# JuliaMLTools/GraphNets.jl

Measured on AMD Instinct MI355X. Metric: edges updated/sec, GNBlock fwd, 1M-edge batch, higher is better.
Workload: dtype f32; 1 GPU; C2: one shared Erdos-Renyi graph, 100k nodes / 1M edges, batch_size=1 (BASELINE configs[1]); dims=(10, 5, 0)=>(3, 4, 5), edges_whole_job=1000000, edges_per_gpu=1000000, nodes_per_gpu=100000, graphs_per_gpu=1, parallelism=single GPU

## Files before the change

graphnets.jl_amd/csrc/gnx_forward.hip:

```cpp
#include <algorithm>
#include <cstdlib>

#include "gnx_staging.h"
#include "gnx_step_hazard.h"

namespace gnx {

static_assert(GNX_ACT_IDENTITY == 0 && GNX_ACT_RELU == 1 && GNX_ACT_TANH == 2 && GNX_ACT_SIGMOID == 3 && GNX_ACT_GELU == 4,
              "act_apply (gnx_device.h) hard-codes the activation codes");

static int32_t check_block(const gnx_graphs* h, const gnx_block_params* p, int64_t R) {
  if (!h || !p) return fail(GNX_ERR_INVALID_ARG, "NULL handle or params");
  if (R <= 0) return fail(GNX_ERR_INVALID_ARG, "n_replicas must be >= 1");
  if (R > 1 && h->G != 1)
    return fail(GNX_ERR_INVALID_ARG, "n_replicas > 1 needs a single-graph handle (shared adjacency, batch.jl:66)");
  if (R > 65535) return fail(GNX_ERR_TOO_LARGE, "n_replicas exceeds the grid limit (65535)");
  const int d[6] = {p->de, p->dn, p->dg, p->oe, p->on, p->og};
  for (int i = 0; i < 6; ++i)
    if (d[i] < 0) return fail(GNX_ERR_DIMS, "negative feature width");
  if (p->de + p->dn + p->dg == 0) return fail(GNX_ERR_DIMS, "all input widths are 0 (gnblock.jl:48, batch.jl:56)");
  if (p->oe + p->on + p->og == 0) return fail(GNX_ERR_DIMS, "all output widths are 0 (gnblock.jl:49)");
  const gnx_dense* fn[3] = {&p->edgefn, &p->nodefn, &p->graphfn};
  const int out[3] = {p->oe, p->on, p->og};
  const int in[3] = {p->de + 2 * p->dn + p->dg, p->oe + p->dn + p->dg, p->oe + p->on + p->dg};
// ... 309 lines not shown
  int32_t rc = bf16 ? check_call(c) : GNX_OK;
  if (rc) return rc;
  if (prev && prev->workspace && (prev->workspace == c.ws || (c.p && c.p->og > 0 && prev->gf_out == c.gf_out)))
    return fail(GNX_ERR_INVALID_ARG, bf16 ? "internal: the pending step's workspace / gf_out is this step's"
                                          : "the pending call's workspace / gf_out must not be this call's (its graph update has not run yet)");
  bool took = false;
  rc = block_chained(c.on(c.s, GNX_PHASE_EDGE_NODE), prev, took);
  if (rc) return rc;
  if (took) {
    *pending = gnx_pending_update{c.ws, c.ws_bytes, static_cast<const float*>(c.gf), static_cast<float*>(c.gf_out)};
    return GNX_OK;
  }
  if (prev && prev->workspace) {
    rc = graph_update(c.h, c.p, c.elem, *prev, c.R, c.flags, c.s);
    if (rc) return rc;
  }
  *pending = gnx_pending_update{};
  return bf16 ? gnx_block_forward_typed(c.h, c.p, GNX_ELEM_BF16, c.ef, c.nf, c.gf, c.R, c.ef_out, c.nf_out, c.gf_out, c.ws, c.ws_bytes, c.flags, c.s) : block_plain(c);
}

int32_t gnx_block_forward_chained(const gnx_graphs* h, const gnx_block_params* p, const float* ef, const float* nf, const float* gf, int64_t R, float* ef_out,
                                  float* nf_out, float* gf_out, void* ws, size_t ws_bytes, uint32_t flags, void* stream, const gnx_pending_update* prev,
                                  gnx_pending_update* pending) {
  if (!pending) return fail(GNX_ERR_INVALID_ARG, "pending is NULL");
  DeviceTurn turn((hipStream_t)stream, p && matrix_core_widths(*p));
  if (flags & GNX_FLAG_DEFER_GRAPH_UPDATE) return fail(GNX_ERR_INVALID_ARG, "gnx_block_forward_chained defers the graph update itself");
  return chained_step(BlockCall{h, p, GNX_ELEM_F32, ef, nf, gf, R, ef_out, nf_out, gf_out, ws, ws_bytes, flags, (hipStream_t)stream, GNX_PHASE_ALL}, prev, pending);
}

static StepSpans step_spans(const gnx_graphs* h, const gnx_block_params* p, int64_t R, const gnx_block_step& st, size_t elem, size_t ws_extent) {
  const void* const in[3] = {st.ef, st.nf, st.gf};
  const void* const out[3] = {st.ef_out, st.nf_out, st.gf_out};
  const long long rows[3] = {(long long)h->E, (long long)h->N, (long long)h->G};
  const int in_w[3] = {p->de, p->dn, p->dg}, out_w[3] = {p->oe, p->on, p->og};
  return step_spans_of(in, out, st.workspace, st.workspace_bytes, rows, in_w, out_w, R, elem, ws_extent);
}

static bool steps_overlap_applies(const gnx_graphs* h, const gnx_block_params* p, int64_t R, uint32_t flags, hipStream_t s) {
  if (!h || !p || matrix_core_widths(*p) || (flags & GNX_FLAG_FORCE_GENERIC) || form(GNX_FLAG_NO_FORK) || profile_enabled()) return false;
  if (check_block(h, p, R) != GNX_OK) return false;
  return block_narrow_takes(h, block_probe(h, p), s);
}

constexpr int kStepsRunDefault = 8;
static_assert(kRunMax == kRunSlots, "gnx_step_hazard.h groups what gnx_device.h's table holds");
static int steps_run_max() {
  static const int v = [] {
    const char* e = getenv("GNX_STEPS_RUN_MAX");
    const int n = e && *e ? atoi(e) : kStepsRunDefault;
    return n < 1 ? 1 : (n > kRunMax ? kRunMax : n);
  }();
  return v;
}

static int32_t steps_schedule(const gnx_graphs* h, const gnx_block_params* p, int32_t elem, const gnx_block_step* steps, int64_t n_steps, int64_t R,
                              uint32_t flags, void* stream, bool overlap) {
  const AuxHold hold = overlap ? take_aux(h, true) : AuxHold{};
  const gnx_graphs::AuxSet* aux = hold.set;
  const bool two = aux != nullptr;
  hipStream_t str[2] = {(hipStream_t)stream, aux ? aux->stream : nullptr};
  gnx_pending_update pend[2]{};
  auto flush = [&](int k) -> int32_t {
    if (!pend[k].workspace) return GNX_OK;
    const int32_t rc = graph_update(h, p, elem, pend[k], R, flags, str[k]);
    pend[k] = gnx_pending_update{};
    return rc;
  };
  auto run = [&](const gnx_block_step& st, int k, gnx_pending_update* next) -> int32_t {
    const gnx_pending_update* prev = pend[k].workspace ? &pend[k] : nullptr;
    return chained_step(BlockCall{h, p, elem, st.ef, st.nf, st.gf, R, st.ef_out, st.nf_out, st.gf_out, st.workspace, st.workspace_bytes, flags, str[k], GNX_PHASE_ALL},
                        prev, next);
  };
  const bool bf16 = elem == GNX_ELEM_BF16;
  const bool valid = h && p && check_block(h, p, R) == GNX_OK;
  const size_t elem_bytes = bf16 ? 2 : sizeof(float);
  const size_t ws_extent = !valid ? 0 : bf16 ? typed_ws(h, p, R, true).total : block_ws(h, p, R).total;
  bool can_fuse = valid && R == 1 && !(flags & GNX_FLAG_FORCE_GENERIC) && steps_run_max() > 1 && !profile_enabled();
  auto slot_of = [&](const gnx_block_step& st, RunSlot& sl, BlockArgs* run_args) -> bool {
    Prepared q(BlockCall{h, p, elem, st.ef, st.nf, st.gf, R, st.ef_out, st.nf_out, st.gf_out, st.workspace, st.workspace_bytes, flags, str[0], GNX_PHASE_ALL});
    if (q.rc) return false;
    if (run_args) {
      if (!block_narrow_run_applies(h, q.a, bf16)) return can_fuse = false;
      *run_args = q.a;
    }
    sl = RunSlot{q.a.ef, q.a.nf, q.a.gf, q.a.ef_out, q.a.nf_out, q.a.gf_out, q.a.partials};
    return true;
  };
  if (two) {
    GNX_HIP(hipEventRecord(aux->fork, str[0]));
    GNX_HIP(hipStreamWaitEvent(str[1], aux->fork, 0));
  }
  RunSpans recent[3];
  int32_t rc = GNX_OK;
  int64_t i = 0;
  for (int64_t j = 0; i < n_steps && rc == GNX_OK; ++j) {
    const gnx_block_step& st = steps[i];
    RunSpans cur;
    RunTable tab{};
    BlockArgs run_args{};
    cur.step[0] = valid ? step_spans(h, p, R, st, elem_bytes, ws_extent) : StepSpans{};
    cur.n = 1;
    if (can_fuse && n_steps - i >= 2) {
      RunSpans win = cur;
      while (i + win.n < n_steps) {
        const StepSpans sp = step_spans(h, p, R, steps[i + win.n], elem_bytes, ws_extent);
        if (!run_takes(win, sp, steps_run_max())) break;
        win.step[win.n++] = sp;
      }
      bool ok = window_is_run(win.n, i, n_steps, steps_run_max());
      for (int z = 0; ok && z < win.n; ++z) ok = slot_of(steps[i + z], tab.slot[z], z == 0 ? &run_args : nullptr);
      if (ok) cur = win;
    }
    const int k = two ? (int)(j & 1) : 0, o = k ^ 1;
    StepOrder ord;
    if (two) {
      ord = run_order(cur, recent, j);
    } else {
      ord.flush_own = pend[0].workspace && (pend[0].workspace == st.workspace || (p && p->og > 0 && pend[0].gf_out == st.gf_out) || runs_conflict(cur, recent[0]));
    }
    if ((ord.flush_own || cur.n > 1) && (rc = flush(k))) break;
    if (two && j >= 3) {
      const hipError_t e = hipStreamWaitEvent(str[k], aux->step[(j - 3) & 3], 0);
      if (e != hipSuccess) { rc = hip_fail(e, "gnx_block_forward_steps: ordering a step behind the step three before it"); break; }
    }
    if (ord.after_other) {
      if ((rc = flush(o))) break;
      hipEvent_t ev = o == 1 ? aux->join : aux->fork;
      hipError_t e = hipEventRecord(ev, str[o]);
      if (e == hipSuccess) e = hipStreamWaitEvent(str[k], ev, 0);
      if (e != hipSuccess) { rc = hip_fail(e, "gnx_block_forward_steps: ordering a step behind the other stream"); break; }
    }
    if (cur.n > 1) {
      rc = launch_block_narrow_run(h, run_args, tab, cur.n, str[k], bf16);
    } else {
      gnx_pending_update next{};
      rc = run(st, k, &next);
      if (rc == GNX_OK) pend[k] = next;
    }
    if (rc != GNX_OK) break;
    if (two) {
      if (const hipError_t e = hipEventRecord(aux->step[j & 3], str[k]); e != hipSuccess) { rc = hip_fail(e, "gnx_block_forward_steps: step event"); break; }
    }
    recent[2] = recent[1]; recent[1] = recent[0]; recent[0] = cur;
    i += cur.n;
  }
  const int32_t rf0 = flush(0), rf1 = two ? flush(1) : GNX_OK;
  hipError_t e1 = hipSuccess, e2 = hipSuccess;
  if (two) {
    e1 = hipEventRecord(aux->join, str[1]);
    e2 = hipStreamWaitEvent(str[0], aux->join, 0);
  }
  if (rc) return rc;
  if (rf0) return rf0;
  if (rf1) return rf1;
  GNX_HIP(e1);
  GNX_HIP(e2);
  return GNX_OK;
}

int32_t gnx_block_forward_steps(const gnx_graphs* h, const gnx_block_params* p, const gnx_block_step* steps, int64_t n_steps, int64_t R, uint32_t flags,
                                void* stream) {
  if (n_steps < 0 || (n_steps > 0 && !steps)) return fail(GNX_ERR_INVALID_ARG, "gnx_block_forward_steps: steps is NULL / n_steps is negative");
  if (flags & GNX_FLAG_DEFER_GRAPH_UPDATE) return fail(GNX_ERR_INVALID_ARG, "gnx_block_forward_steps finishes every step's graph update itself");
  DeviceTurn turn((hipStream_t)stream, p && matrix_core_widths(*p));
  FormScope forms(flags);
  return steps_schedule(h, p, GNX_ELEM_F32, steps, n_steps, R, flags, stream, n_steps > 1 && steps_overlap_applies(h, p, R, flags, (hipStream_t)stream));
}

int32_t gnx_block_forward_steps_typed(const gnx_graphs* h, const gnx_block_params* p, int32_t elem, const gnx_block_step* steps, int64_t n_steps, int64_t R,
                                      uint32_t flags, void* stream) {
  if (elem == GNX_ELEM_F32) return gnx_block_forward_steps(h, p, steps, n_steps, R, flags, stream);
  if (elem != GNX_ELEM_BF16) return fail(GNX_ERR_INVALID_ARG, "elem must be GNX_ELEM_F32 or GNX_ELEM_BF16");
  if (flags & GNX_FLAG_DEFER_GRAPH_UPDATE) return fail(GNX_ERR_INVALID_ARG, "gnx_block_forward_steps_typed finishes every step's graph update itself");
  if (n_steps < 0 || (n_steps > 0 && !steps)) return fail(GNX_ERR_INVALID_ARG, "gnx_block_forward_steps_typed: steps is NULL / n_steps is negative");
  for (int64_t i = 0; i < n_steps; ++i) {
    const gnx_block_step& st = steps[i];
    const void* bufs[6] = {st.ef, st.nf, st.gf, st.ef_out, st.nf_out, st.gf_out};
    for (const void* b : bufs)
      if (((uintptr_t)b & 3) != 0) return fail(GNX_ERR_INVALID_ARG, "bf16 feature buffers must be 4-byte aligned (in every step)");
  }
  const hipStream_t s = (hipStream_t)stream;
  DeviceTurn turn(s, p && matrix_core_widths(*p));
  FormScope forms(flags);
  if (!h || !p || check_block(h, p, R) != GNX_OK || !typed_native(h, p, flags, s)) {
    for (int64_t i = 0; i < n_steps; ++i) {
      const gnx_block_step& st = steps[i];
      if (int32_t rc = gnx_block_forward_typed(h, p, GNX_ELEM_BF16, st.ef, st.nf, st.gf, R, st.ef_out, st.nf_out, st.gf_out, st.workspace, st.workspace_bytes,
                                               flags, stream))
        return rc;
    }
    return GNX_OK;
  }
  return steps_schedule(h, p, GNX_ELEM_BF16, steps, n_steps, R, flags, stream, n_steps > 1 && !form(GNX_FLAG_NO_FORK) && !profile_enabled());
}

int32_t gnx_block_graph_update(const gnx_graphs* h, const gnx_block_params* p, const float* gf, int64_t R, float* gf_out, void* ws,
                               size_t ws_bytes, uint32_t flags, void* stream) {
  return graph_update(h, p, GNX_ELEM_F32, gnx_pending_update{ws, ws_bytes, gf, gf_out}, R, flags, (hipStream_t)stream);
}

static int partial_rows_of(const gnx_graphs* h) { return (int)(h->G == 1 ? (h->n_wtiles() + 3) / 4 : h->n_wtiles()); }

static bool ffn_on_mfma(int d) { return d >= 32; }

struct CoreLayout {
  size_t ln1[3], ln2[3], hidden, block, total;
  float* at(void* ws, size_t off) const { return reinterpret_cast<float*>(static_cast<char*>(ws) + off); }
  float* gn1(void* ws, int t) const { return at(ws, ln1[t]); }
  float* gn2(void* ws, int t) const { return at(ws, ln2[t]); }
  float* stats(void* ws, int t) const { return gn1(ws, t); }
  float* x6_planes(void* ws, int t) const { return gn2(ws, t); }
  float* block_out(void* ws, int t) const { return gn1(ws, t); }
};
static CoreLayout core_layout(const gnx_graphs* h, const gnx_core_params* p, int64_t R) {
  const size_t rows[3] = {(size_t)R * h->E, (size_t)R * h->N, (size_t)R * h->G};
  const int d[3] = {p->block.de, p->block.dn, p->block.dg};
  CoreLayout L{};
  size_t o = 0, hidden = 0;
  for (int t = 0; t < 3; ++t) {
    L.ln1[t] = o; o += align_up(sizeof(float) * rows[t] * d[t], 256);
    L.ln2[t] = o; o += align_up(sizeof(float) * rows[t] * d[t], 256);
    if (ffn_on_mfma(d[t])) hidden = std::max(hidden, sizeof(float) * rows[t] * 4 * (size_t)d[t]);
  }
  L.hidden = o; o += align_up(hidden, 256);
  L.block = o;
  L.total = o + block_ws(h, &p->block, R).total;
  return L;
}

static int32_t check_core_dims(const gnx_block_params& b) {
  if (b.de <= 0 || b.dn <= 0 || b.dg <= 0) return fail(GNX_ERR_DIMS, "GNCore needs all(dims .> 0) (gnfeedforward.jl:18)");
  if (b.oe != b.de || b.on != b.dn || b.og != b.dg) return fail(GNX_ERR_DIMS, "GNCore's block must map dims => dims (gncore.jl:49)");
  return GNX_OK;
}
static int32_t check_core(const gnx_graphs* h, const gnx_core_params* p, const gnx_block_params& b, int64_t R, const void* ef, const void* nf, const void* gf,
                          const void* ef_out, const void* nf_out, const void* gf_out, uint32_t flags) {
  int32_t rc = check_core_dims(b);
  if (rc) return rc;
  rc = check_block(h, &b, R);
  if (rc) return rc;
  if (((!ef || !ef_out) && h->E > 0) || !nf || !gf || !nf_out || !gf_out) return fail(GNX_ERR_INVALID_ARG, "GNCore needs ef, nf, gf and all outputs");
  for (int t = 0; t < 3; ++t) {
    if (!p->ln1[t].gamma || !p->ln1[t].beta || !p->ln2[t].gamma || !p->ln2[t].beta) return fail(GNX_ERR_INVALID_ARG, "LayerNorm parameter is NULL");
    if (!p->ff[t].fc1.weight || !p->ff[t].fc2.weight) return fail(GNX_ERR_INVALID_ARG, "FeedForward weight is NULL");
  }
  if (p->eps_mode != 0 && p->eps_mode != 1) return fail(GNX_ERR_INVALID_ARG, "eps_mode must be 0 or 1");
  const int dd[3] = {b.de, b.dn, b.dg};
  for (int t = 0; t < 3; ++t) {
    const bool generic = !ffn_on_mfma(dd[t]) || (flags & (GNX_FLAG_FORCE_GENERIC | GNX_FLAG_NO_MFMA));
    if (generic && (size_t)dd[t] * 5 * 4 * sizeof(float) > 64 * 1024)
      return fail(GNX_ERR_DIMS, "GNCore width too large for the generic FFN kernel (80*d bytes of LDS)");
  }
  return GNX_OK;
}
// ... 347 lines not shown
```

graphnets.jl_amd/csrc/gnx_launchers.h:

```cpp
#pragma once
#include "gnx_internal.h"

namespace gnx {

struct EdgeLaunch {
  const Tile* tiles; size_t n_tiles; const float* ef; size_t E;
  struct { const float* stats; const float* g; const float* b; bool inline_stats; float eps; int mode; } ln;
  const float* We; int ldw;
  const float* psrc;
  const float* pdst;
  size_t N; const int* src; const int* dst; int act;
  float* out; float* colsum;
  float* agg_out; size_t n_agg_rows; const int* chunk_row0;
  int64_t R; void* scratch; hipStream_t stream;
};

int32_t launch_block_generic(const BlockArgs& a, int64_t R, int tile_n_cap, hipStream_t s, int phase);
int32_t launch_layernorm2(const float* x, size_t rows, int d, const gnx_layernorm& l1, const gnx_layernorm& l2, float eps, int eps_mode, float* y1, float* y2, hipStream_t s);
int32_t launch_layernorm2_bf16(const void* x, size_t rows, int d, const gnx_layernorm& l1, const gnx_layernorm& l2, float eps, int eps_mode, float* y1, float* y2, hipStream_t s);
int32_t launch_ffn_residual(const float* z, const float* x, size_t rows, int d, const gnx_ffn& ff, float* out, hipStream_t s);
int32_t launch_pad(const gnx_graphs* h, int kind, bool pad, const float* src, int d, int64_t R, float* dst, hipStream_t s);
int32_t launch_calibration(int n, hipStream_t s);
int xent_blocks(int64_t cols);
int32_t launch_xent_backward(const float* logits, const float* targets, int d, int64_t cols, const float* upstream, float* dl, hipStream_t s);
int32_t launch_xent(const float* logits, const float* targets, int d, int64_t cols, float* out, float* ws, hipStream_t s);
int32_t launch_collapse(const gnx_graphs* h, const float* ef, int d, int64_t R, float* out, hipStream_t s);
int32_t launch_collapse_padded(const gnx_graphs* h, const float* ef, int d, int64_t R, float* out, hipStream_t s);
int32_t launch_fn_input(const gnx_graphs* h, int kind, const float* ef, int de, const float* nf, int dn, const float* gf, int dg, int64_t R, float* out, hipStream_t s,
                        bool bf16 = false);

int32_t launch_block_narrow(const gnx_graphs* h, const BlockArgs& a, int64_t R, hipStream_t s, int phase, bool bf16 = false);
void warm_block_narrow(const gnx_graphs* h, const gnx_block_params* p, bool bf16 = false);
bool block_narrow_ready(const gnx_graphs* h, const BlockArgs& a, hipStream_t s);
bool block_narrow_ffe_applies(const gnx_graphs* h, const BlockArgs& a, int act1, int act2);
bool block_narrow_chain_applies(const gnx_graphs* h, const BlockArgs& a, bool bf16 = false);
bool block_narrow_takes(const gnx_graphs* h, const BlockArgs& a, hipStream_t s, bool bf16 = false);
int32_t launch_block_narrow_chained(const gnx_graphs* h, const BlockArgs& a, int64_t R, hipStream_t s, bool bf16);
bool narrow_bf16_aot(const gnx_graphs* h, const BlockArgs& a);
int32_t launch_fused_bf16(const gnx_graphs* h, const BlockArgs& a, int64_t R, hipStream_t s, int phase);
int32_t launch_chained_bf16(const gnx_graphs* h, const BlockArgs& a, int64_t R, hipStream_t s);
bool narrow_bf16_ln_aot(const gnx_graphs* h, const BlockArgs& a);
int32_t launch_ln_bf16(const gnx_graphs* h, const BlockArgs& a, int64_t R, hipStream_t s, int phase);
bool block_narrow_run_applies(const gnx_graphs* h, const BlockArgs& a, bool bf16);
bool narrow_bf16_run(const gnx_graphs* h, const BlockArgs& a);
int32_t launch_block_narrow_run(const gnx_graphs* h, const BlockArgs& a, const RunTable& t, int Z, hipStream_t s, bool bf16);
int32_t launch_run_bf16(const gnx_graphs* h, const BlockArgs& a, const RunTable& t, int Z, hipStream_t s);
bool jit_eligible(const BlockArgs& a, int ept);
int32_t jit_get(const BlockArgs& a, int ept, hipStream_t s, hipFunction_t* block, hipFunction_t* graph, bool bf16 = false);
int32_t jit_get_core_post3(int d0, int d1, int d2, hipStream_t s, hipFunction_t* fn);

bool core_narrow_width(int d);
int32_t launch_ln1_rows(const float* x, size_t rows, int d, const gnx_layernorm& l1, float eps, int eps_mode, float* y, hipStream_t s);
bool core_post3_applies(const size_t rows[3], const int d[3], const gnx_ffn ff[3], bool deferred, hipStream_t s);
int32_t launch_core_post3(const float* const x[3], const size_t rows[3], const int d[3], const gnx_layernorm l2[3], const gnx_ffn ff[3], float eps,
                          int eps_mode, float* const out[3], hipStream_t s, const BlockArgs* blk, int n_rows, bool skip_edges = false,
                          const float* const block_out[3] = nullptr);
int32_t launch_core_post(const float* x, size_t rows, int d, const gnx_layernorm& l2, const gnx_ffn& ff, float eps, int eps_mode, float* out, hipStream_t s,
                         const float* block_out = nullptr);

int32_t launch_block_wide(const gnx_graphs* h, const BlockArgs& a, int64_t R, hipStream_t s, int phase);
size_t wide_workspace_bytes(const gnx_graphs* h, const gnx_block_params* p, int64_t R);
void warm_block_wide(const gnx_graphs* h, const gnx_block_params* p, bool rows_gemm);
bool block_wide_ln_applies(const gnx_graphs* h, const BlockArgs& a);
bool block_wide_edge_x6_applies(const gnx_graphs* h, const BlockArgs& a);
int32_t launch_dense_rows(const gnx_graphs* h, int entity, const float* A, int K, const gnx_dense& d, int OUT, const float* add1,
                          const float* add2, float* out, int64_t R, hipStream_t s, const char* name);
int32_t launch_rows_matmul(const gnx_graphs* h, int entity, const float* A, int K, const float* B, int ldw, int OUT, float* out, int64_t R,
                           hipStream_t s, const char* name, const float* gmul, int gmul_act, float* tile_colsum, int* n_tiles_out, const float* add1);

int32_t launch_ffn_fused(const gnx_graphs* h, int entity, const float* z, int d, const gnx_ffn& ff, const float* add1, const float* add2, float* out,
                         int64_t R, hipStream_t s, const float* ln_stats = nullptr, const gnx_layernorm* ln = nullptr, void* scratch = nullptr, size_t scratch_bytes = 0,
                         bool ln_inline = false, float ln_eps = 0.f, int ln_mode = 0);
bool ffn_fused_applies(const float* z, int d, const gnx_ffn& ff, const float* add1, const float* add2, const float* out);
bool ln_stats_applies(const float* x, int d);
int32_t launch_ln_stats(const float* x, size_t rows, int d, float eps, int eps_mode, float* stats, hipStream_t s);
bool ffn_x6_applies(const float* z, int d, const gnx_ffn& ff, const float* add1, const float* add2, const float* out, size_t scratch_bytes);
int32_t launch_ffn_x6(const float* z, size_t nrows, int d, const gnx_ffn& ff, const float* add1, const float* add2, float* out, int64_t R, hipStream_t s,
                      const float* ln_stats, const gnx_layernorm* ln, void* scratch, bool ln_inline, float ln_eps, int ln_mode);
int32_t launch_ffn_x6_prep(const float* W1, const float* W2, int d, void* scratch, hipStream_t s, const float* ln_gamma, const float* ln_beta, const float* b1);
size_t ffn_x6_scratch_bytes(int d);
size_t ffn_x6_fold_scratch_bytes(int d);
int32_t launch_core_edge_x6(const EdgeLaunch& e, const gnx_ffn& ff, const gnx_layernorm* ln2, void* scratch_f);

int32_t launch_edge_x6(const EdgeLaunch& e, int oe);
int32_t launch_edge_x6_prep(const float* We, int ldw, void* scratch, hipStream_t s, int n_out, const float* ln_gamma, const float* ln_beta);
size_t edge_x6_scratch_bytes();
size_t edge_x6_fold_scratch_bytes();
int32_t launch_fold_beta(const float* W, int ldw, int K, int n_out, const float* beta, const float* bias, float* out, hipStream_t s);
bool proj_x6_applies(int dn, int oe, const float* nf, const float* W, const float* out, size_t N);
int32_t launch_proj_x6(const Tile* tiles, size_t n_tiles, const float* nf, size_t N, const float* ln_stats, const float* ln_g, const float* ln_b, const float* Ws, const float* Wd,
                       int ldw, const float* bias, const float* bias_g, int G, float* out_s, float* out_d, int64_t R, void* scratch, hipStream_t s, bool only_d = false,
                       float* zn_out = nullptr);
int32_t launch_proj_x6_prep(const float* Ws, const float* Wd, int ldw, void* scratch, hipStream_t s);
size_t proj_x6_scratch_bytes();
int32_t launch_edge_enc(const EdgeLaunch& e, const float* bias, const float* bias_g, int G);
int32_t launch_edge_enc_prep(const float* We, int ldw, void* scratch, hipStream_t s);
size_t edge_enc_scratch_bytes();
bool node_x6_applies(int oe, int dn, int on, int act, const float* nf, const float* Wn, const float* out, size_t N);
int32_t launch_node_x6(const Tile* tiles, size_t n_tiles, const float* nf, size_t N, const float* ln_stats, const float* ln_g, const float* ln_b, const float* agg,
// ... 50 lines not shown
```

graphnets.jl_amd/csrc/gnx_narrow.hip:

```cpp
#include <cstdlib>

#include "gnx_launchers.h"
#include "gnx_narrow_launch.h"
#include "gnx_wave_kernel.h"

namespace gnx {

#define GNX_NARROW_DIMS(X) \
  X(10, 5, 0, 3, 4)        \
  X(3, 4, 5, 3, 4)         \
  X(10, 5, 3, 3, 4)        \
  X(0, 2, 0, 2, 2)         \
  X(2, 2, 2, 2, 2)         \
  X(4, 3, 2, 3, 4)         \
  X(8, 8, 8, 16, 8)        \
  X(10, 5, 3, 10, 5)       \
  X(10, 5, 0, 10, 5)
static bool narrow_aot_listed(const BlockArgs& a) {
#define GNX_CASE(DE, DN, DG, OE, ON) \
  if (a.de == DE && a.dn == DN && a.dg == DG && a.oe == OE && a.on == ON) return true;
  GNX_NARROW_DIMS(GNX_CASE)
#undef GNX_CASE
  return false;
}
// ... 48 lines not shown
  } else if (narrow_aot_listed(a)) {
    return h->wtile_e_cap == 64 || h->wtile_e_cap == 128 || h->wtile_e_cap == 256;
  }
  const int ept = jit_ept(h);
  hipFunction_t fb, fg;
  return ept && jit_get(a, ept, s, &fb, &fg) == GNX_OK;
}

static bool pack_form(const gnx_graphs* h, const BlockArgs& a) { return h->G > 1 && h->n_packs > 0 && a.packs && a.og > 0 && !getenv("GNX_NO_PACK"); }
bool block_narrow_chain_applies(const gnx_graphs* h, const BlockArgs& a, bool bf16) {
  if (a.n_wtiles == 0 || a.E == 0 || a.og <= 0 || h->wtile_e_cap != 128 || wants_ln(a) || a.ffe_w1 || pack_form(h, a)) return false;
  const int C = a.oe + a.on;
  if (C <= 0) return false;
  const int wsl = wave_slice_floats(a.oe, 2);
  if (h->G == 1) { if (graph_update_lds_floats(C, a.dg, a.og, graph_update_threads(h)) > 4 * wsl) return false; }
  else if (h->max_wtiles_per_graph > 256 || graph_update_lds_floats(C, a.dg, a.og, 64) > wsl) return false;
  return narrow_aot_listed(a) && (!bf16 || narrow_bf16_aot(h, a));
}
int32_t launch_block_narrow_chained(const gnx_graphs* h, const BlockArgs& a0, int64_t R, hipStream_t s, bool bf16) {
  BlockArgs a = a0;
  a.prev_blocks = a.prev_partials ? (h->G == 1 ? 1 : (int)((h->G + 3) / 4)) : 0;
  if (bf16) {
    const int32_t rc = launch_chained_bf16(h, a, R, s);
    return rc == 1 ? fail(GNX_ERR_INVALID_ARG, "internal: chained bf16 launch for a width set without that kernel") : rc;
  }
#define GNX_CASE(DE, DN, DG, OE, ON)                                                                                               \
  if (a.de == DE && a.dn == DN && a.dg == DG && a.oe == OE && a.on == ON) {                                                         \
    if constexpr (OE + ON > 0) {                                                                                                   \
      return h->G == 1 ? launch_wave_g<DE, DN, DG, OE, ON, 2, false, true, false, true>(h, a, R, s, 1)                              \
                       : launch_wave_g<DE, DN, DG, OE, ON, 2, false, false, false, true>(h, a, R, s, 1);                            \
    }                                                                                                                              \
  }
  GNX_NARROW_DIMS(GNX_CASE)
#undef GNX_CASE
  return fail(GNX_ERR_INVALID_ARG, "internal: chained launch for a width set without that kernel");
}

#define GNX_NARROW_RUN_DIMS(X) \
  X(10, 5, 0, 3, 4)            \
  X(3, 4, 5, 3, 4)             \
  X(10, 5, 3, 3, 4)            \
  X(0, 2, 0, 2, 2)             \
  X(2, 2, 2, 2, 2)             \
  X(4, 3, 2, 3, 4)
bool block_narrow_run_applies(const gnx_graphs* h, const BlockArgs& a, bool bf16) {
  if (!block_narrow_chain_applies(h, a, bf16)) return false;
  if (bf16) return narrow_bf16_run(h, a);
#define GNX_CASE(DE, DN, DG, OE, ON) \
  if (a.de == DE && a.dn == DN && a.dg == DG && a.oe == OE && a.on == ON) return true;
  GNX_NARROW_RUN_DIMS(GNX_CASE)
#undef GNX_CASE
  return false;
}
int32_t launch_block_narrow_run(const gnx_graphs* h, const BlockArgs& a, const RunTable& t, int Z, hipStream_t s, bool bf16) {
  if (bf16) {
    const int32_t rc = launch_run_bf16(h, a, t, Z, s);
    return rc == 1 ? fail(GNX_ERR_INVALID_ARG, "internal: bf16 run launch for a width set without that kernel") : rc;
  }
#define GNX_CASE(DE, DN, DG, OE, ON)                                                                                               \
  if (a.de == DE && a.dn == DN && a.dg == DG && a.oe == OE && a.on == ON) {                                                         \
    if constexpr (OE + ON > 0) {                                                                                                   \
      return h->G == 1 ? launch_wave_run<DE, DN, DG, OE, ON, true>(h, a, t, Z, s) : launch_wave_run<DE, DN, DG, OE, ON, false>(h, a, t, Z, s); \
    }                                                                                                                              \
  }
  GNX_NARROW_RUN_DIMS(GNX_CASE)
#undef GNX_CASE
  return fail(GNX_ERR_INVALID_ARG, "internal: run launch for a width set without that kernel");
}

bool block_narrow_ffe_applies(const gnx_graphs* h, const BlockArgs& a, int act1, int act2) {
  return ln_aot(h, a) && a.ln_g[0] && act1 <= GNX_ACT_RELU && act2 <= GNX_ACT_RELU && a.act_e <= GNX_ACT_RELU && h->max_in_degree <= h->wtile_e_cap &&
         !form(GNX_FLAG_NO_FFE);
}

enum NarrowRoute { NR_NONE, NR_AOT, NR_JIT };
static NarrowRoute narrow_route(const gnx_graphs* h, const BlockArgs& a, hipStream_t s, bool bf16 = false) {
  if (a.n_wtiles == 0 || a.E == 0 || wants_ln(a)) return NR_NONE;
  auto jit_ok = [&]() {
    const int ept = jit_ept(h);
    hipFunction_t fb, fg;
    return ept && jit_get(a, ept, s, &fb, &fg, bf16) == GNX_OK;
  };
  static const bool jit_all = getenv("GNX_JIT_ALL") != nullptr;
  if (jit_all && jit_ok()) return NR_JIT;
  if (bf16) {
    if (narrow_bf16_aot(h, a)) return NR_AOT;
  } else if (narrow_aot_listed(a)) {
    return h->wtile_e_cap == 64 || h->wtile_e_cap == 128 || (h->wtile_e_cap == 256 && (a.de + a.dn) * 4 <= 64) ? NR_AOT : NR_NONE;
  }
  return jit_ok() ? NR_JIT : NR_NONE;
}

bool block_narrow_takes(const gnx_graphs* h, const BlockArgs& a, hipStream_t s, bool bf16) { return narrow_route(h, a, s, bf16) != NR_NONE; }

int32_t launch_block_narrow(const gnx_graphs* h, const BlockArgs& a, int64_t R, hipStream_t s, int phase, bool bf16) {
  if (a.n_wtiles == 0 || a.E == 0) return 1;
  if (wants_ln(a)) {
    if (bf16) {
      const int32_t rc = launch_ln_bf16(h, a, R, s, phase);
      return rc == 1 ? fail(GNX_ERR_INVALID_ARG, "internal: LayerNorm-on-load on bf16 rows for a width set without that kernel") : rc;
    }
    if (a.ffe_w1) {
      if (!ln_aot(h, a)) return fail(GNX_ERR_INVALID_ARG, "internal: FeedForward-in-the-edge-lanes requested for a width set without that kernel");
      return h->G == 1 ? launch_wave_g<10, 5, 3, 10, 5, 2, true, true, true>(h, a, R, s, phase) : launch_wave_g<10, 5, 3, 10, 5, 2, true, false, true>(h, a, R, s, phase);
    }
    if (ln_aot(h, a)) return launch_wave_t<10, 5, 3, 10, 5, 2, true>(h, a, R, s, phase);
    const int32_t rc = launch_wave_jit(h, a, R, s, phase);
    return rc == 1 ? fail(GNX_ERR_INVALID_ARG, "internal: LayerNorm-on-load requested but the fused kernel is not available") : rc;
  }
  const NarrowRoute route = narrow_route(h, a, s, bf16);
  if (route == NR_NONE) return 1;
  if (route == NR_JIT) return launch_wave_jit(h, a, R, s, phase, bf16);
  if (bf16) {
    const int32_t rc = launch_fused_bf16(h, a, R, s, phase);
    return rc == 1 ? fail(GNX_ERR_INVALID_ARG, "internal: ahead-of-time bf16 route for a width set without that kernel") : rc;
// ... 10 lines not shown
```

graphnets.jl_amd/csrc/gnx_narrow_bf16.hip:

```cpp
#include "gnx_launchers.h"
#include "gnx_narrow_launch.h"
#include "gnx_wave_kernel.h"

namespace gnx {

#define GNX_NARROW_DIMS_BF16(X) \
  X(10, 5, 0, 3, 4)             \
  X(3, 4, 5, 3, 4)

bool narrow_bf16_aot(const gnx_graphs* h, const BlockArgs& a) {
#define GNX_CASE(DE, DN, DG, OE, ON)                                     \
  if (a.de == DE && a.dn == DN && a.dg == DG && a.oe == OE && a.on == ON) \
    return h->wtile_e_cap == 64 || h->wtile_e_cap == 128 || (h->wtile_e_cap == 256 && (DE + DN) * 4 <= 64);
  GNX_NARROW_DIMS_BF16(GNX_CASE)
#undef GNX_CASE
  return false;
}

int32_t launch_fused_bf16(const gnx_graphs* h, const BlockArgs& a, int64_t R, hipStream_t s, int phase) {
#define GNX_CASE(DE, DN, DG, OE, ON) \
  if (a.de == DE && a.dn == DN && a.dg == DG && a.oe == OE && a.on == ON) return launch_fused<DE, DN, DG, OE, ON, true>(h, a, R, s, phase);
  GNX_NARROW_DIMS_BF16(GNX_CASE)
#undef GNX_CASE
  return 1;
}

int32_t launch_chained_bf16(const gnx_graphs* h, const BlockArgs& a, int64_t R, hipStream_t s) {
#define GNX_CASE(DE, DN, DG, OE, ON)                                                                                               \
  if (a.de == DE && a.dn == DN && a.dg == DG && a.oe == OE && a.on == ON) {                                                         \
    if constexpr (OE + ON > 0) {                                                                                                   \
      return h->G == 1 ? launch_wave_g<DE, DN, DG, OE, ON, 2, false, true, false, true, true>(h, a, R, s, 1)                        \
                       : launch_wave_g<DE, DN, DG, OE, ON, 2, false, false, false, true, true>(h, a, R, s, 1);                      \
    }                                                                                                                              \
  }
  GNX_NARROW_DIMS_BF16(GNX_CASE)
#undef GNX_CASE
  return 1;
}

bool narrow_bf16_ln_aot(const gnx_graphs* h, const BlockArgs& a) {
  return a.n_wtiles > 0 && a.E > 0 && a.de == 10 && a.dn == 5 && a.dg == 3 && a.oe == 10 && a.on == 5 && h->wtile_e_cap == 128;
}
int32_t launch_ln_bf16(const gnx_graphs* h, const BlockArgs& a, int64_t R, hipStream_t s, int phase) {
  if (!narrow_bf16_ln_aot(h, a)) return 1;
  if (a.ffe_w1)
    return h->G == 1 ? launch_wave_g<10, 5, 3, 10, 5, 2, true, true, true, false, true>(h, a, R, s, phase)
                     : launch_wave_g<10, 5, 3, 10, 5, 2, true, false, true, false, true>(h, a, R, s, phase);
  return launch_wave_t<10, 5, 3, 10, 5, 2, true, true>(h, a, R, s, phase);
}

#define GNX_NARROW_RUN_DIMS_BF16(X) \
  X(10, 5, 0, 3, 4, false)          \
  X(3, 4, 5, 3, 4, true)
bool narrow_bf16_run(const gnx_graphs* h, const BlockArgs& a) {
#define GNX_CASE(DE, DN, DG, OE, ON, SEVERAL) \
  if (a.de == DE && a.dn == DN && a.dg == DG && a.oe == OE && a.on == ON) return h->G == 1 || SEVERAL;
  GNX_NARROW_RUN_DIMS_BF16(GNX_CASE)
#undef GNX_CASE
  return false;
}
int32_t launch_run_bf16(const gnx_graphs* h, const BlockArgs& a, const RunTable& t, int Z, hipStream_t s) {
#define GNX_CASE(DE, DN, DG, OE, ON, SEVERAL)                                                                \
  if (a.de == DE && a.dn == DN && a.dg == DG && a.oe == OE && a.on == ON) {                                   \
    if (h->G == 1) return launch_wave_run<DE, DN, DG, OE, ON, true, true>(h, a, t, Z, s);                     \
    if constexpr (SEVERAL) return launch_wave_run<DE, DN, DG, OE, ON, false, true>(h, a, t, Z, s);            \
  }
  GNX_NARROW_RUN_DIMS_BF16(GNX_CASE)
#undef GNX_CASE
  return 1;
}

}
```

graphnets.jl_amd/csrc/gnx_narrow_launch.h:

```cpp
#pragma once
#include <cstdlib>

#include "gnx_device.h"
#include "gnx_wave_kernel.h"

namespace gnx {

static int partial_rows(const gnx_graphs* h) { return (int)(h->G == 1 ? (h->n_wtiles() + 3) / 4 : h->n_wtiles()); }

static int graph_update_threads(const gnx_graphs* h) {
  return graph_update_threads_for_rows(h->G == 1 ? (h->n_wtiles() + 3) / 4 : h->max_wtiles_per_graph);
}

template <int DE, int DN, int DG, int OE, int ON, int EPT, bool LN, bool ONEG, bool FFE = false, bool CHAIN = false, bool BF16 = false>
static int32_t launch_wave_g(const gnx_graphs* h, const BlockArgs& a, int64_t R, hipStream_t s, int phase) {
  constexpr int C = OE + ON;
  const int n_rows = partial_rows(h);
  const unsigned grid = (unsigned)((a.n_wtiles + 3) / 4) + (CHAIN ? (unsigned)a.prev_blocks : 0u);
  if (phase & 1) {
    ProfScope ps("k_block_wave", s);
#ifdef GNX_WAVE_STAMPS_BUILD
    static unsigned long long* d_dbg = nullptr;
    static size_t dbg_cap = 0;
    const char* dump = getenv("GNX_WAVE_STAMPS_DUMP");
    if (dump) {
      if (dbg_cap < (size_t)a.n_wtiles) { if (d_dbg) (void)hipFree(d_dbg); dbg_cap = (size_t)a.n_wtiles; (void)hipMalloc((void**)&d_dbg, dbg_cap * 64); }
      (void)hipMemsetAsync(d_dbg, 0, (size_t)a.n_wtiles * 64, s);
      (void)hipMemcpyToSymbolAsync(HIP_SYMBOL(g_wave_dbg), &d_dbg, sizeof(d_dbg), 0, hipMemcpyHostToDevice, s);
    }
#endif
    if constexpr (FFE) GNX_LAUNCH((k_block_wave_ffe<DE, DN, DG, OE, ON, EPT, ONEG, BF16>), dim3(grid, (unsigned)R), dim3(kThreads), 0, s, a, n_rows);
    else GNX_LAUNCH((k_block_wave<DE, DN, DG, OE, ON, EPT, LN, ONEG, false, false, CHAIN, BF16>), dim3(grid, (unsigned)R), dim3(kThreads), 0, s, a, n_rows);
    GNX_HIP(hipGetLastError());
#ifdef GNX_WAVE_STAMPS_BUILD
    if (dump) {
      (void)hipStreamSynchronize(s);
      std::vector<unsigned long long> hs((size_t)a.n_wtiles * 8);
      (void)hipMemcpy(hs.data(), d_dbg, hs.size() * 8, hipMemcpyDeviceToHost);
      if (FILE* f = fopen(dump, "wb")) { fwrite(hs.data(), 8, hs.size(), f); fclose(f); }
    }
#endif
  }
  if ((phase & 2) && a.og > 0) {
    if constexpr (C > 0) {
      const int threads = graph_update_threads(h);
      const size_t lds = sizeof(float) * (size_t)graph_update_lds_floats(C, a.dg, a.og, threads);
      ProfScope ps("k_graph_t", s);
      GNX_LAUNCH((k_graph_t<C, ONEG, BF16, BF16 && !LN>), dim3((unsigned)a.G, (unsigned)R), dim3(threads), lds, s, a, n_rows);
      GNX_HIP(hipGetLastError());
    }
  }
  return GNX_OK;
}

template <int DE, int DN, int DG, int OE, int ON, bool ONEG, bool BF16 = false>
static int32_t launch_wave_run(const gnx_graphs* h, const BlockArgs& a, const RunTable& t, int Z, hipStream_t s) {
  constexpr int C = OE + ON;
  if (Z < 1 || Z > kRunSlots) return fail(GNX_ERR_INVALID_ARG, "internal: a run of more steps than the table has slots");
  const int n_rows = partial_rows(h);
  {
    ProfScope ps("k_block_wave", s);
    GNX_LAUNCH((k_block_wave_run<DE, DN, DG, OE, ON, 2, ONEG, BF16>), dim3((unsigned)((a.n_wtiles + 3) / 4), (unsigned)Z), dim3(kThreads), 0, s, a, t, n_rows);
    GNX_HIP(hipGetLastError());
  }
  if (a.og > 0) {
    const int threads = graph_update_threads(h);
    const size_t lds = sizeof(float) * (size_t)graph_update_lds_floats(C, a.dg, a.og, threads);
    ProfScope ps("k_graph_t", s);
    GNX_LAUNCH((k_graph_run<C, ONEG, BF16>), dim3((unsigned)a.G, (unsigned)Z), dim3(threads), lds, s, a, t, n_rows);
    GNX_HIP(hipGetLastError());
  }
  return GNX_OK;
}

template <int DE, int DN, int DG, int OE, int ON, int EPT, bool BF16 = false>
static bool launch_wave_pack(const gnx_graphs* h, const BlockArgs& a, int64_t R, hipStream_t s, int phase, int32_t* rc) {
  constexpr int C = OE + ON;
  if constexpr (EPT != 2 || C == 0) return false;
  else {
    if (h->G <= 1 || h->n_packs <= 0 || !a.packs || phase != 3 || a.og <= 0 || form(GNX_FLAG_NO_PACK)) return false;
    ProfScope ps("k_block_wave", s);
    GNX_LAUNCH((k_block_wave<DE, DN, DG, OE, ON, EPT, false, false, true, false, false, BF16>), dim3((unsigned)h->n_packs, (unsigned)R), dim3(kPackThreads), 0, s, a, 0);
    const hipError_t e = hipGetLastError();
    *rc = e == hipSuccess ? GNX_OK : hip_fail(e, "k_block_wave<PACK>");
    return true;
  }
}

template <int DE, int DN, int DG, int OE, int ON, int EPT, bool LN = false, bool BF16 = false>
static int32_t launch_wave_t(const gnx_graphs* h, const BlockArgs& a, int64_t R, hipStream_t s, int phase) {
  if constexpr (!LN) {
    int32_t rc = GNX_OK;
    if (launch_wave_pack<DE, DN, DG, OE, ON, EPT, BF16>(h, a, R, s, phase, &rc)) return rc;
  }
  return h->G == 1 ? launch_wave_g<DE, DN, DG, OE, ON, EPT, LN, true, false, false, BF16>(h, a, R, s, phase)
                   : launch_wave_g<DE, DN, DG, OE, ON, EPT, LN, false, false, false, BF16>(h, a, R, s, phase);
}

template <int DE, int DN, int DG, int OE, int ON, bool BF16 = false>
static int32_t launch_fused(const gnx_graphs* h, const BlockArgs& a, int64_t R, hipStream_t s, int phase) {
  if (h->wtile_e_cap == 64) return launch_wave_t<DE, DN, DG, OE, ON, 1, false, BF16>(h, a, R, s, phase);
  if (h->wtile_e_cap == 128) return launch_wave_t<DE, DN, DG, OE, ON, 2, false, BF16>(h, a, R, s, phase);
  if (h->wtile_e_cap == 256) {
    if constexpr ((DE + DN) * 4 <= 64) return launch_wave_t<DE, DN, DG, OE, ON, 4, false, BF16>(h, a, R, s, phase);
  }
  return 1;
}

}
```

graphnets.jl_amd/csrc/gnx_step_hazard.h:

```cpp
#pragma once
#include <cstddef>
#include <cstdint>

namespace gnx {

struct ByteSpan {
  uintptr_t lo = 0, hi = 0;
};

inline ByteSpan byte_span(const void* p, size_t bytes) {
  ByteSpan s;
  if (p && bytes) { s.lo = reinterpret_cast<uintptr_t>(p); s.hi = s.lo + bytes; }
  return s;
}

inline bool spans_overlap(ByteSpan a, ByteSpan b) { return a.lo < a.hi && b.lo < b.hi && a.lo < b.hi && b.lo < a.hi; }

struct StepSpans {
  ByteSpan rd[3];
  ByteSpan wr[4];
};

inline StepSpans step_spans_of(const void* const in[3], const void* const out[3], const void* ws, size_t ws_bytes, const long long rows[3],
                               const int in_w[3], const int out_w[3], long long R, size_t elem, size_t ws_extent) {
// ... 22 lines not shown
  bool after_other = false;
};
inline StepOrder step_order(const StepSpans& cur, const StepSpans* recent, long long i) {
  StepOrder o;
  o.flush_own = i >= 2 && steps_conflict(cur, recent[1]);
  o.after_other = (i >= 1 && steps_conflict(cur, recent[0])) || (i >= 3 && steps_conflict(cur, recent[2]));
  return o;
}

constexpr int kRunMax = 8;
constexpr int kRunTailMin = 4;

struct RunSpans {
  int n = 0;
  StepSpans step[kRunMax];
};

inline bool run_conflicts_step(const RunSpans& r, const StepSpans& s) {
  for (int a = 0; a < r.n; ++a)
    if (steps_conflict(r.step[a], s)) return true;
  return false;
}

inline bool runs_conflict(const RunSpans& x, const RunSpans& y) {
  for (int b = 0; b < y.n; ++b)
    if (run_conflicts_step(x, y.step[b])) return true;
  return false;
}

inline bool run_takes(const RunSpans& run, const StepSpans& next, int run_max) {
  return run.n >= 1 && run.n < run_max && run.n < kRunMax && !run_conflicts_step(run, next);
}

inline bool window_is_run(int n, long long first, long long n_steps, int run_max) {
  return n >= 2 && (n == run_max || (first + n == n_steps && n >= kRunTailMin));
}

inline RunSpans group_run(const StepSpans* spans, long long n_steps, long long first, int run_max) {
  RunSpans run;
  if (first >= n_steps) return run;
  run.step[run.n++] = spans[first];
  while (first + run.n < n_steps && run_takes(run, spans[first + run.n], run_max)) { run.step[run.n] = spans[first + run.n]; ++run.n; }
  if (!window_is_run(run.n, first, n_steps, run_max)) run.n = 1;
  return run;
}

inline StepOrder run_order(const RunSpans& cur, const RunSpans* recent, long long j) {
  StepOrder o;
  o.flush_own = j >= 2 && runs_conflict(cur, recent[1]);
  o.after_other = (j >= 1 && runs_conflict(cur, recent[0])) || (j >= 3 && runs_conflict(cur, recent[2]));
  return o;
}

}
```

Measured before the change: 58.16 billion edges/s.

## Overlap a fused run's graph-update launch with the next run's block kernel

Fused multi-step runs are split into a block launch and a graph-update launch. The graph update of the previous run is held back and issued on the other stream beside the next run's block kernel. Each run alternates between two partials homes in the workspace, so consecutive runs do not collide; a new hazard check confirms the per-launch read/write spans are disjoint. This aims to hide the small graph-reduction kernel behind edge/node work. The cost is more events and cross-stream waits, and a more intricate ordering that must stay correct.

```diff
diff --git a/graphnets.jl_amd/csrc/gnx_forward.hip b/graphnets.jl_amd/csrc/gnx_forward.hip
--- a/graphnets.jl_amd/csrc/gnx_forward.hip
+++ b/graphnets.jl_amd/csrc/gnx_forward.hip
@@ -385,6 +385,8 @@
   }();
   return v;
 }
+
+static int partial_rows_of(const gnx_graphs* h) { return (int)(h->G == 1 ? (h->n_wtiles() + 3) / 4 : h->n_wtiles()); }
 
 static int32_t steps_schedule(const gnx_graphs* h, const gnx_block_params* p, int32_t elem, const gnx_block_step* steps, int64_t n_steps, int64_t R,
                               uint32_t flags, void* stream, bool overlap) {
@@ -423,6 +425,41 @@
     GNX_HIP(hipEventRecord(aux->fork, str[0]));
     GNX_HIP(hipStreamWaitEvent(str[1], aux->fork, 0));
   }
+  const size_t home_bytes = valid ? sizeof(float) * (size_t)partial_rows_of(h) * (size_t)((p->oe + p->on + 3) / 4 * 4) : 0;
+  const BlockWs ws_lay = valid ? block_ws(h, p, R) : BlockWs{};
+  const size_t home_off[2] = {ws_lay.part_off, ws_lay.agg_off};
+  const bool second_home = valid && p->og > 0 && home_bytes > 0 && ws_lay.agg_off + home_bytes <= ws_lay.part_off;
+  struct Held {
+    bool has = false;
+    BlockArgs args{};
+    RunTable tab{};
+    int n = 0, k = 0, home = 0;
+    int64_t j = 0;
+    RunLaunches launches;
+  } held;
+  bool train = false;
+  auto behind = [&](int to, int from, const char* what) -> int32_t {
+    hipEvent_t ev = from == 1 ? aux->join : aux->fork;
+    hipError_t e = hipEventRecord(ev, str[from]);
+    if (e == hipSuccess) e = hipStreamWaitEvent(str[to], ev, 0);
+    return e == hipSuccess ? GNX_OK : hip_fail(e, what);
+  };
+  int step_on[4] = {0, 0, 0, 0};
+  enum Place { kBehind, kBeside, kLast };
+  auto place_held = [&](Place where) -> int32_t {
+    if (!held.has) return GNX_OK;
+    held.has = false;
+    const int g = where == kBeside ? held.k ^ 1 : held.k;
+    hipError_t e = hipSuccess;
+    if (where == kBeside) e = hipStreamWaitEvent(str[g], held.k == 1 ? aux->join : aux->fork, 0);
+    if (where == kLast) e = hipStreamWaitEvent(str[g], aux->step[(held.j - 1) & 3], 0);
+    if (e != hipSuccess) return hip_fail(e, "gnx_block_forward_steps: ordering a run's graph updates");
+    const int32_t r = launch_block_narrow_run(h, held.args, held.tab, held.n, str[g], bf16, kRunGraph);
+    if (r != GNX_OK || !two) return r;
+    e = hipEventRecord(aux->step[held.j & 3], str[g]);
+    step_on[held.j & 3] = g;
+    return e == hipSuccess ? GNX_OK : hip_fail(e, "gnx_block_forward_steps: step event");
+  };
   RunSpans recent[3];
   int32_t rc = GNX_OK;
   int64_t i = 0;
@@ -444,6 +481,54 @@
       for (int z = 0; ok && z < win.n; ++z) ok = slot_of(steps[i + z], tab.slot[z], z == 0 ? &run_args : nullptr);
       if (ok) cur = win;
     }
+    RunLaunches cur_l;
+    int home = 0;
+    bool relaxed = false;
+    if (cur.n > 1) {
+      const int other = run_home(true, held.home);
+      if (two && held.has && (other == 0 || second_home) && runs_conflict(cur, recent[0])) {
+        cur_l = run_launches(cur, home_off[other], home_bytes);
+        relaxed = run_relaxed_after(held.launches, cur_l);
+      }
+      home = run_home(relaxed, held.home);
+      if (!relaxed) cur_l = run_launches(cur, home_off[0], home_bytes);
+      if (home != 0)
+        for (int z = 0; z < cur.n; ++z) tab.slot[z].partials = reinterpret_cast<float*>(static_cast<char*>(steps[i + z].workspace) + home_off[home]);
+    }
+    if (relaxed) {
+      const int b = held.k, g = b ^ 1;
+      const int64_t before = held.j;
+      if (!train) {
+        if ((rc = flush(g))) break;
+        if ((rc = behind(b, g, "gnx_block_forward_steps: ordering a train of runs behind the other stream"))) break;
+      }
+      if (const hipError_t e = hipEventRecord(b == 1 ? aux->join : aux->fork, str[b]); e != hipSuccess) { rc = hip_fail(e, "gnx_block_forward_steps: event behind a block launch"); break; }
+      if (train) {
+        if (const hipError_t e = hipStreamWaitEvent(str[b], aux->step[(before - 1) & 3], 0); e != hipSuccess) {
+          rc = hip_fail(e, "gnx_block_forward_steps: ordering a block launch behind the graph updates two runs before it");
+          break;
+        }
+      }
+      const int32_t rb = launch_block_narrow_run(h, run_args, tab, cur.n, str[b], bf16, kRunBlock);
+      if ((rc = place_held(kBeside))) break;
+      if ((rc = rb)) break;
+      held.has = true; held.args = run_args; held.tab = tab; held.n = cur.n; held.k = b; held.home = home; held.j = j; held.launches = cur_l;
+      train = true;
+      recent[2] = recent[1]; recent[1] = recent[0]; recent[0] = cur;
+      i += cur.n;
+      continue;
+    }
+    if (held.has) {
+      const int b = held.k;
+      if (train) {
+        if (const hipError_t e = hipEventRecord(b == 1 ? aux->join : aux->fork, str[b]); e != hipSuccess) { rc = hip_fail(e, "gnx_block_forward_steps: event behind a block launch"); break; }
+        if ((rc = place_held(kBeside))) break;
+        if ((rc = behind(b, b ^ 1, "gnx_block_forward_steps: joining the streams after a train of runs"))) break;
+      } else if ((rc = place_held(kBehind))) {
+        break;
+      }
+      train = false;
+    }
     const int k = two ? (int)(j & 1) : 0, o = k ^ 1;
     StepOrder ord;
     if (two) {
@@ -452,7 +537,7 @@
       ord.flush_own = pend[0].workspace && (pend[0].workspace == st.workspace || (p && p->og > 0 && pend[0].gf_out == st.gf_out) || runs_conflict(cur, recent[0]));
     }
     if ((ord.flush_own || cur.n > 1) && (rc = flush(k))) break;
-    if (two && j >= 3) {
+    if (two && j >= 3 && step_on[(j - 3) & 3] != k) {
       const hipError_t e = hipStreamWaitEvent(str[k], aux->step[(j - 3) & 3], 0);
       if (e != hipSuccess) { rc = hip_fail(e, "gnx_block_forward_steps: ordering a step behind the step three before it"); break; }
     }
@@ -464,19 +549,22 @@
       if (e != hipSuccess) { rc = hip_fail(e, "gnx_block_forward_steps: ordering a step behind the other stream"); break; }
     }
     if (cur.n > 1) {
-      rc = launch_block_narrow_run(h, run_args, tab, cur.n, str[k], bf16);
+      rc = launch_block_narrow_run(h, run_args, tab, cur.n, str[k], bf16, kRunBlock);
+      if (rc == GNX_OK) { held.has = true; held.args = run_args; held.tab = tab; held.n = cur.n; held.k = k; held.home = 0; held.j = j; held.launches = cur_l; }
     } else {
       gnx_pending_update next{};
       rc = run(st, k, &next);
       if (rc == GNX_OK) pend[k] = next;
     }
     if (rc != GNX_OK) break;
-    if (two) {
+    if (two && cur.n == 1) {
       if (const hipError_t e = hipEventRecord(aux->step[j & 3], str[k]); e != hipSuccess) { rc = hip_fail(e, "gnx_block_forward_steps: step event"); break; }
+      step_on[j & 3] = k;
     }
     recent[2] = recent[1]; recent[1] = recent[0]; recent[0] = cur;
     i += cur.n;
   }
+  const int32_t rh = place_held(train ? kLast : kBehind);
   const int32_t rf0 = flush(0), rf1 = two ? flush(1) : GNX_OK;
   hipError_t e1 = hipSuccess, e2 = hipSuccess;
   if (two) {
@@ -484,6 +572,7 @@
     e2 = hipStreamWaitEvent(str[0], aux->join, 0);
   }
   if (rc) return rc;
+  if (rh) return rh;
   if (rf0) return rf0;
   if (rf1) return rf1;
   GNX_HIP(e1);
@@ -531,8 +620,6 @@
                                size_t ws_bytes, uint32_t flags, void* stream) {
   return graph_update(h, p, GNX_ELEM_F32, gnx_pending_update{ws, ws_bytes, gf, gf_out}, R, flags, (hipStream_t)stream);
 }
-
-static int partial_rows_of(const gnx_graphs* h) { return (int)(h->G == 1 ? (h->n_wtiles() + 3) / 4 : h->n_wtiles()); }
 
 static bool ffn_on_mfma(int d) { return d >= 32; }
 
diff --git a/graphnets.jl_amd/csrc/gnx_launchers.h b/graphnets.jl_amd/csrc/gnx_launchers.h
--- a/graphnets.jl_amd/csrc/gnx_launchers.h
+++ b/graphnets.jl_amd/csrc/gnx_launchers.h
@@ -43,8 +43,9 @@
 int32_t launch_ln_bf16(const gnx_graphs* h, const BlockArgs& a, int64_t R, hipStream_t s, int phase);
 bool block_narrow_run_applies(const gnx_graphs* h, const BlockArgs& a, bool bf16);
 bool narrow_bf16_run(const gnx_graphs* h, const BlockArgs& a);
-int32_t launch_block_narrow_run(const gnx_graphs* h, const BlockArgs& a, const RunTable& t, int Z, hipStream_t s, bool bf16);
-int32_t launch_run_bf16(const gnx_graphs* h, const BlockArgs& a, const RunTable& t, int Z, hipStream_t s);
+enum : int { kRunBlock = 1, kRunGraph = 2, kRunBoth = 3 };
+int32_t launch_block_narrow_run(const gnx_graphs* h, const BlockArgs& a, const RunTable& t, int Z, hipStream_t s, bool bf16, int parts = kRunBoth);
+int32_t launch_run_bf16(const gnx_graphs* h, const BlockArgs& a, const RunTable& t, int Z, hipStream_t s, int parts);
 bool jit_eligible(const BlockArgs& a, int ept);
 int32_t jit_get(const BlockArgs& a, int ept, hipStream_t s, hipFunction_t* block, hipFunction_t* graph, bool bf16 = false);
 int32_t jit_get_core_post3(int d0, int d1, int d2, hipStream_t s, hipFunction_t* fn);
diff --git a/graphnets.jl_amd/csrc/gnx_narrow.hip b/graphnets.jl_amd/csrc/gnx_narrow.hip
--- a/graphnets.jl_amd/csrc/gnx_narrow.hip
+++ b/graphnets.jl_amd/csrc/gnx_narrow.hip
@@ -124,15 +124,15 @@
 #undef GNX_CASE
   return false;
 }
-int32_t launch_block_narrow_run(const gnx_graphs* h, const BlockArgs& a, const RunTable& t, int Z, hipStream_t s, bool bf16) {
+int32_t launch_block_narrow_run(const gnx_graphs* h, const BlockArgs& a, const RunTable& t, int Z, hipStream_t s, bool bf16, int parts) {
   if (bf16) {
-    const int32_t rc = launch_run_bf16(h, a, t, Z, s);
+    const int32_t rc = launch_run_bf16(h, a, t, Z, s, parts);
     return rc == 1 ? fail(GNX_ERR_INVALID_ARG, "internal: bf16 run launch for a width set without that kernel") : rc;
   }
 #define GNX_CASE(DE, DN, DG, OE, ON)                                                                                               \
   if (a.de == DE && a.dn == DN && a.dg == DG && a.oe == OE && a.on == ON) {                                                         \
     if constexpr (OE + ON > 0) {                                                                                                   \
-      return h->G == 1 ? launch_wave_run<DE, DN, DG, OE, ON, true>(h, a, t, Z, s) : launch_wave_run<DE, DN, DG, OE, ON, false>(h, a, t, Z, s); \
+      return h->G == 1 ? launch_wave_run<DE, DN, DG, OE, ON, true>(h, a, t, Z, s, parts) : launch_wave_run<DE, DN, DG, OE, ON, false>(h, a, t, Z, s, parts); \
     }                                                                                                                              \
   }
   GNX_NARROW_RUN_DIMS(GNX_CASE)
diff --git a/graphnets.jl_amd/csrc/gnx_narrow_bf16.hip b/graphnets.jl_amd/csrc/gnx_narrow_bf16.hip
--- a/graphnets.jl_amd/csrc/gnx_narrow_bf16.hip
+++ b/graphnets.jl_amd/csrc/gnx_narrow_bf16.hip
@@ -59,11 +59,11 @@
 #undef GNX_CASE
   return false;
 }
-int32_t launch_run_bf16(const gnx_graphs* h, const BlockArgs& a, const RunTable& t, int Z, hipStream_t s) {
+int32_t launch_run_bf16(const gnx_graphs* h, const BlockArgs& a, const RunTable& t, int Z, hipStream_t s, int parts) {
 #define GNX_CASE(DE, DN, DG, OE, ON, SEVERAL)                                                                \
   if (a.de == DE && a.dn == DN && a.dg == DG && a.oe == OE && a.on == ON) {                                   \
-    if (h->G == 1) return launch_wave_run<DE, DN, DG, OE, ON, true, true>(h, a, t, Z, s);                     \
-    if constexpr (SEVERAL) return launch_wave_run<DE, DN, DG, OE, ON, false, true>(h, a, t, Z, s);            \
+    if (h->G == 1) return launch_wave_run<DE, DN, DG, OE, ON, true, true>(h, a, t, Z, s, parts);              \
+    if constexpr (SEVERAL) return launch_wave_run<DE, DN, DG, OE, ON, false, true>(h, a, t, Z, s, parts);     \
   }
   GNX_NARROW_RUN_DIMS_BF16(GNX_CASE)
 #undef GNX_CASE
diff --git a/graphnets.jl_amd/csrc/gnx_narrow_launch.h b/graphnets.jl_amd/csrc/gnx_narrow_launch.h
--- a/graphnets.jl_amd/csrc/gnx_narrow_launch.h
+++ b/graphnets.jl_amd/csrc/gnx_narrow_launch.h
@@ -54,16 +54,16 @@
 }
 
 template <int DE, int DN, int DG, int OE, int ON, bool ONEG, bool BF16 = false>
-static int32_t launch_wave_run(const gnx_graphs* h, const BlockArgs& a, const RunTable& t, int Z, hipStream_t s) {
+static int32_t launch_wave_run(const gnx_graphs* h, const BlockArgs& a, const RunTable& t, int Z, hipStream_t s, int parts) {
   constexpr int C = OE + ON;
   if (Z < 1 || Z > kRunSlots) return fail(GNX_ERR_INVALID_ARG, "internal: a run of more steps than the table has slots");
   const int n_rows = partial_rows(h);
-  {
+  if (parts & kRunBlock) {
     ProfScope ps("k_block_wave", s);
     GNX_LAUNCH((k_block_wave_run<DE, DN, DG, OE, ON, 2, ONEG, BF16>), dim3((unsigned)((a.n_wtiles + 3) / 4), (unsigned)Z), dim3(kThreads), 0, s, a, t, n_rows);
     GNX_HIP(hipGetLastError());
   }
-  if (a.og > 0) {
+  if ((parts & kRunGraph) && a.og > 0) {
     const int threads = graph_update_threads(h);
     const size_t lds = sizeof(float) * (size_t)graph_update_lds_floats(C, a.dg, a.og, threads);
     ProfScope ps("k_graph_t", s);
diff --git a/graphnets.jl_amd/csrc/gnx_step_hazard.h b/graphnets.jl_amd/csrc/gnx_step_hazard.h
--- a/graphnets.jl_amd/csrc/gnx_step_hazard.h
+++ b/graphnets.jl_amd/csrc/gnx_step_hazard.h
@@ -98,4 +98,80 @@
   return o;
 }
 
+struct RunLaunches {
+  int n = 0;
+  ByteSpan in[kRunMax][3];
+  ByteSpan out[kRunMax][3];
+  ByteSpan ws[kRunMax];
+  ByteSpan home[kRunMax];
+};
+
+inline RunLaunches run_launches(const RunSpans& r, size_t home_off, size_t home_bytes) {
+  RunLaunches L;
+  L.n = r.n;
+  for (int a = 0; a < r.n; ++a) {
+    for (int t = 0; t < 3; ++t) { L.in[a][t] = r.step[a].rd[t]; L.out[a][t] = r.step[a].wr[t]; }
+    L.ws[a] = r.step[a].wr[3];
+    const ByteSpan w = L.ws[a];
+    if (w.lo < w.hi && home_bytes > 0 && home_off <= w.hi - w.lo && home_bytes <= w.hi - w.lo - home_off) { L.home[a].lo = w.lo + home_off; L.home[a].hi = L.home[a].lo + home_bytes; }
+  }
+  return L;
 }
+
+enum RunLaunch { kLaunchBlock = 0, kLaunchGraph = 1 };
+struct LaunchAccess {
+  int nr = 0, nw = 0;
+  ByteSpan rd[3 * kRunMax], wr[3 * kRunMax];
+};
+inline LaunchAccess launch_access(const RunLaunches& L, RunLaunch which) {
+  LaunchAccess x;
+  for (int a = 0; a < L.n; ++a) {
+    if (which == kLaunchBlock) {
+      for (int t = 0; t < 3; ++t) x.rd[x.nr++] = L.in[a][t];
+      x.wr[x.nw++] = L.out[a][0]; x.wr[x.nw++] = L.out[a][1]; x.wr[x.nw++] = L.home[a];
+    } else {
+      x.rd[x.nr++] = L.home[a]; x.rd[x.nr++] = L.in[a][2];
+      x.wr[x.nw++] = L.out[a][2];
+    }
+  }
+  return x;
+}
+inline bool launches_conflict(const LaunchAccess& x, const LaunchAccess& y) {
+  for (int i = 0; i < x.nw; ++i) {
+    for (int k = 0; k < y.nr; ++k) if (spans_overlap(x.wr[i], y.rd[k])) return true;
+    for (int k = 0; k < y.nw; ++k) if (spans_overlap(x.wr[i], y.wr[k])) return true;
+  }
+  for (int i = 0; i < y.nw; ++i)
+    for (int k = 0; k < x.nr; ++k) if (spans_overlap(y.wr[i], x.rd[k])) return true;
+  return false;
+}
+
+inline bool run_relaxed_after(const RunLaunches& prev, const RunLaunches& cur) {
+  if (prev.n < 2 || cur.n < 2) return false;
+  const RunLaunches* const both[2] = {&prev, &cur};
+  for (int x = 0; x < 2; ++x)
+    for (int a = 0; a < both[x]->n; ++a) {
+      const ByteSpan h = both[x]->home[a], w = both[x]->ws[a];
+      if (!(h.lo < h.hi)) return false;
+      for (int y = 0; y < 2; ++y)
+        for (int b = 0; b < both[y]->n; ++b) {
+          for (int t = 0; t < 3; ++t)
+            if (spans_overlap(h, both[y]->in[b][t]) || spans_overlap(h, both[y]->out[b][t])) return false;
+          if (x == y && a == b) continue;
+          const ByteSpan v = both[y]->ws[b];
+          const bool same_ws = v.lo == w.lo && v.hi == w.hi;
+          if (spans_overlap(w, v) && !(same_ws && x != y)) return false;
+          if (spans_overlap(h, both[y]->home[b])) return false;
+        }
+    }
+  const LaunchAccess blk = launch_access(cur, kLaunchBlock);
+  for (int a = 0; a < prev.n; ++a) {
+    for (int k = 0; k < blk.nr; ++k) if (spans_overlap(prev.out[a][2], blk.rd[k])) return false;
+    for (int k = 0; k < blk.nw; ++k) if (spans_overlap(prev.out[a][2], blk.wr[k])) return false;
+  }
+  return !launches_conflict(launch_access(prev, kLaunchGraph), blk);
+}
+
+inline int run_home(bool relaxed, int prev_home) { return relaxed ? prev_home ^ 1 : 0; }
+
+}
```

New measurement: 54.47 billion edges/s. 0.937x the previous value.
